# zillow/salve

Hardware: AMD Instinct MI355X
Metric: alignment hypotheses/sec (render+verify) (higher is better)
Workload: dtype fp16

## Files before the change

### include/salve_hip.h

```cpp
#ifndef SALVE_HIP_H
#define SALVE_HIP_H

#include <stddef.h>
#include <stdint.h>

#ifdef __cplusplus
extern "C" {
#endif

typedef enum {
    SALVE_OK = 0,
    SALVE_ERR_BAD_ARG = -1,
    SALVE_ERR_UNSUPPORTED = -2,
    SALVE_ERR_HIP = -3,
    SALVE_ERR_WORKSPACE = -4
} salve_status_t;

#define SALVE_HIP_ABI_VERSION 7

#define SALVE_STATUS_WALK_FAILED 1
#define SALVE_STATUS_FP16_RANGE 2
#define SALVE_STATUS_BAD_HYPOTHESIS 4

#define SALVE_STATUS_LAYOUT_THICKNESS 8
// ... 134 lines not shown

typedef struct {
    int32_t op;
    int32_t in_buf, out_buf, res_buf;
    int32_t Hi, Wi, Cin;
    int32_t Ho, Wo, Cout;
    int32_t KH, KW, stride, pad;
    int32_t relu, reserved;
    int64_t w_off;
    int64_t b_off;
    int64_t ktab_off;
    int32_t in2_buf, Cin2, stride2, Hi2, Wi2, reserved2;
} salve_resnet_op_t;

#define SALVE_RESNET_CONV_IGEMM_ONLY 1
#define SALVE_RESNET_CONV8_WHEREVER 2
#define SALVE_RESNET_ROUND_ROBIN_TILES 4
#define SALVE_RESNET_NO_STEM_FUSE 8
#define SALVE_RESNET_NO_BLOCK_FUSE 16
#define SALVE_RESNET_NO_PROJ_FUSE 32
#define SALVE_RESNET_NO_CHAIN 64
#define SALVE_RESNET_CHAIN_EXPAND_ONLY 128
#define SALVE_RESNET_CHAIN_16_WAVES 256
#define SALVE_RESNET_CHAIN_NO_SPLIT 512
#define SALVE_RESNET_CHAIN_STORE_ALL 1024
#define SALVE_RESNET_NO_TRANSPOSED_TILES 2048
#define SALVE_RESNET_NO_NEXT_FUSE 4096
#define SALVE_RESNET_ALL_FLAGS 8191

void* salve_resnet_create(int32_t num_layers, int32_t in_channels, const salve_resnet_op_t* ops, int32_t n_ops,
                          const void* weights_f16, size_t weights_bytes, const float* params_f32, size_t params_bytes,
                          const int32_t* ktab, size_t ktab_entries, int32_t flags);
void salve_resnet_destroy(void* handle);
int salve_resnet_num_layers(void* handle);
size_t salve_resnet_workspace_bytes(void* handle, int32_t batch);
int salve_resnet_forward(void* handle, const void* input, int32_t batch, float* logits, void* workspace,
                         size_t workspace_bytes, int32_t* status, void* stream);

void* salve_resnet_f32_create(int32_t num_layers, int32_t in_channels, const salve_resnet_op_t* ops, int32_t n_ops,
                              const float* weights_f32, size_t weights_bytes, const float* params_f32, size_t params_bytes,
                              const int32_t* ktab, size_t ktab_entries, int32_t flags);
void salve_resnet_f32_destroy(void* handle);
size_t salve_resnet_f32_workspace_bytes(void* handle, int32_t batch);
int salve_resnet_f32_forward(void* handle, const float* input, int32_t batch, float* logits, void* workspace,
                             size_t workspace_bytes, int32_t* status, void* stream);

typedef struct {
    int32_t batch, Hi, Wi, Cin, Ho, Wo, Cout, KH, KW, stride, pad;
} salve_conv_desc_t;
#define SALVE_CONV_FWD 0
#define SALVE_CONV_DGRAD 1
#define SALVE_CONV_WGRAD 2
size_t salve_conv_f32_workspace_bytes(const salve_conv_desc_t* d, int32_t pass);
int salve_conv_f32_forward(const salve_conv_desc_t* d, const float* x, const float* w, float* y, void* ws, size_t ws_bytes, void* stream);
int salve_conv_f32_backward_data(const salve_conv_desc_t* d, const float* dy, const float* w, float* dx, void* ws, size_t ws_bytes,
                                 void* stream);
int salve_conv_f32_backward_weight(const salve_conv_desc_t* d, const float* x, const float* dy, float* dw, void* ws, size_t ws_bytes,
                                   void* stream);

size_t salve_conv_bf16_workspace_bytes(const salve_conv_desc_t* d, int32_t pass);
int salve_conv_bf16_forward(const salve_conv_desc_t* d, const uint16_t* x, const uint16_t* w, uint16_t* y, void* ws, size_t ws_bytes,
                            void* stream);
int salve_conv_bf16_backward_data(const salve_conv_desc_t* d, const uint16_t* dy, const uint16_t* w, uint16_t* dx, void* ws, size_t ws_bytes,
                                  void* stream);
int salve_conv_bf16_backward_weight(const salve_conv_desc_t* d, const uint16_t* x, const uint16_t* dy, float* dw, void* ws, size_t ws_bytes,
                                    void* stream);
// ... 94 lines not shown
```

### salve_amd/_lib.py

```python

from __future__ import annotations

import ctypes
from pathlib import Path

import numpy as np

import os

LIB_PATH = Path(os.environ.get("SALVE_HIP_LIB") or (Path(__file__).resolve().parent / "libsalve_hip.so"))

SALVE_OK = 0
EXPECTED_ABI = 7
TILE_F32_NCHW = 0
TILE_F16_NHWC = 1
TILE_U8X4 = 2
TILE_F32_NHWC = 3
TILE_BF16_NHWC = 4

EXPORTED_SYMBOLS = (
    "salve_hip_version",
    "salve_last_error",
    "salve_bev_workspace_bytes",
    "salve_bev_pano_index_bytes",
    "salve_bev_pano_index_build",
    "salve_bev_render_batch",
    "salve_bev_scatter",
    "salve_bev_densify",
    "salve_bev_scatter_points",
    "salve_zorder_winners",
    "salve_remove_hallucinated",
    "salve_bev_keys_from_pixels",
    "salve_bev_export_u8",
    "salve_layout_rasterise",
    "salve_bev_tiles",
    "salve_bev_tile_pairs",
    "salve_bev_densify_tiles",
    "salve_resize_rgb_u8",
    "salve_resnet_create",
    "salve_resnet_destroy",
    "salve_resnet_workspace_bytes",
    "salve_resnet_forward",
    "salve_resnet_num_layers",
    "salve_resnet_f32_create",
    "salve_resnet_f32_destroy",
    "salve_resnet_f32_workspace_bytes",
    "salve_resnet_f32_forward",
    "salve_bev_tiles_aug",
    "salve_conv_f32_workspace_bytes",
    "salve_conv_f32_forward",
    "salve_conv_f32_backward_data",
    "salve_conv_f32_backward_weight",
    "salve_conv_bf16_workspace_bytes",
    "salve_conv_bf16_forward",
    "salve_conv_bf16_backward_data",
    "salve_conv_bf16_backward_weight",
    "salve_bn_workspace_bytes",
    "salve_bn_f32_forward",
    "salve_bn_f32_backward",
    "salve_bn_bf16_forward",
    "salve_bn_bf16_backward",
    "salve_bev_train_tiles",
    "salve_bev_pano_index_update",
    "salve_layout_pose",
    "salve_adam_step",
    "salve_head_workspace_bytes",
    "salve_head_f32_forward",
    "salve_head_f32_backward",
    "salve_head_bf16_forward",
    "salve_head_bf16_backward",
    "salve_bev_jpeg_roundtrip_workspace_bytes",
    "salve_bev_jpeg_roundtrip",
    "salve_bev_jpeg_encode_workspace_bytes",
    "salve_bev_jpeg_encode_max_bytes",
    "salve_bev_jpeg_encode",
    "salve_bev_jpeg_decode_workspace_bytes",
# ... 113 lines not shown
    lib.salve_bev_densify.argtypes = [ctypes.POINTER(BevConfig), i32, vp, vp, vp, vp, vp, sz, vp]
    lib.salve_bev_densify.restype = ctypes.c_int
    lib.salve_bev_scatter_points.argtypes = [ctypes.POINTER(BevConfig), vp, vp, i32, vp, vp, vp, sz, vp]
    lib.salve_bev_scatter_points.restype = ctypes.c_int
    lib.salve_zorder_winners.argtypes = [vp, vp, vp, i32, vp, i32, i32, i32, vp, vp, vp]
    lib.salve_zorder_winners.restype = ctypes.c_int
    lib.salve_remove_hallucinated.argtypes = [vp, vp, i32, i32, i32, vp, vp, vp]
    lib.salve_remove_hallucinated.restype = ctypes.c_int
    lib.salve_bev_keys_from_pixels.argtypes = [ctypes.POINTER(BevConfig), vp, vp, i32, vp, vp, sz, vp]
    lib.salve_bev_keys_from_pixels.restype = ctypes.c_int
    lib.salve_layout_rasterise.argtypes = [vp, i32, vp, vp, i32, i32, vp, vp, vp]
    lib.salve_layout_rasterise.restype = ctypes.c_int
    f64, i64 = ctypes.c_double, ctypes.c_int64
    lib.salve_layout_pose.argtypes = [vp, vp, i64, vp, vp, vp, i64, i32, vp, i32, f64, f64, f64, i32, vp, vp, i32, vp, i32, vp, vp]
    lib.salve_layout_pose.restype = ctypes.c_int
    lib.salve_bev_export_u8.argtypes = [vp, i32, i32, i32, vp, vp]
    lib.salve_bev_export_u8.restype = ctypes.c_int
    lib.salve_bev_tiles.argtypes = [vp, i32, i32, vp, i32, vp, vp, i32, i32, vp, vp, i32, i32, vp]
    lib.salve_bev_tiles.restype = ctypes.c_int
    lib.salve_bev_tile_pairs.argtypes = [vp, vp, i32, i32, vp, vp, i32, vp, vp, i32, i32, vp, vp, i32, i32, vp]
    lib.salve_bev_tile_pairs.restype = ctypes.c_int
    lib.salve_bev_densify_tiles.argtypes = [ctypes.POINTER(BevConfig), i32, vp, vp, vp, vp, vp, vp, i32, i32, vp, vp, i32, vp, vp, sz, vp]
    lib.salve_bev_densify_tiles.restype = ctypes.c_int
    lib.salve_resize_rgb_u8.argtypes = [vp, i32, i32, i32, vp, i32, i32, vp, vp, vp]
    lib.salve_resize_rgb_u8.restype = ctypes.c_int
    lib.salve_resnet_create.argtypes = [i32, i32, vp, i32, vp, sz, vp, sz, vp, sz, i32]
    lib.salve_resnet_create.restype = vp
    lib.salve_resnet_destroy.argtypes = [vp]
    lib.salve_resnet_destroy.restype = None
    lib.salve_resnet_workspace_bytes.argtypes = [vp, i32]
    lib.salve_resnet_workspace_bytes.restype = sz
    lib.salve_resnet_forward.argtypes = [vp, vp, i32, vp, vp, sz, vp, vp]
    lib.salve_resnet_forward.restype = ctypes.c_int
    lib.salve_resnet_num_layers.argtypes = [vp]
    lib.salve_resnet_num_layers.restype = ctypes.c_int
    lib.salve_resnet_f32_create.argtypes = [i32, i32, vp, i32, vp, sz, vp, sz, vp, sz, i32]
    lib.salve_resnet_f32_create.restype = vp
    lib.salve_resnet_f32_destroy.argtypes = [vp]
    lib.salve_resnet_f32_destroy.restype = None
    lib.salve_resnet_f32_workspace_bytes.argtypes = [vp, i32]
    lib.salve_resnet_f32_workspace_bytes.restype = sz
    lib.salve_resnet_f32_forward.argtypes = [vp, vp, i32, vp, vp, sz, vp, vp]
    lib.salve_resnet_f32_forward.restype = ctypes.c_int
    lib.salve_bev_tiles_aug.argtypes = [vp, i32, i32, vp, vp, i32, vp, vp, i32, i32, vp, vp, i32, vp]
    lib.salve_bev_tiles_aug.restype = ctypes.c_int
    lib.salve_bev_train_tiles.argtypes = [vp, i32, vp, i32, i32, i32, vp, vp, i32, vp, i32, vp, vp, i32, i32, vp, vp, i32, i32, vp, vp]
    lib.salve_bev_train_tiles.restype = ctypes.c_int
    lib.salve_conv_f32_workspace_bytes.argtypes = [ctypes.POINTER(ConvDesc), i32]
    lib.salve_conv_f32_workspace_bytes.restype = sz
    lib.salve_conv_bf16_workspace_bytes.argtypes = [ctypes.POINTER(ConvDesc), i32]
    lib.salve_conv_bf16_workspace_bytes.restype = sz
    for name in ("salve_conv_f32_forward", "salve_conv_f32_backward_data", "salve_conv_f32_backward_weight", "salve_conv_bf16_forward",
                 "salve_conv_bf16_backward_data", "salve_conv_bf16_backward_weight"):
        getattr(lib, name).argtypes = [ctypes.POINTER(ConvDesc), vp, vp, vp, vp, sz, vp]
        getattr(lib, name).restype = ctypes.c_int
    lib.salve_bn_workspace_bytes.argtypes = [ctypes.POINTER(BnDesc), i32]
    lib.salve_bn_workspace_bytes.restype = sz
    for name in ("salve_bn_f32_forward", "salve_bn_bf16_forward"):
        getattr(lib, name).argtypes = [ctypes.POINTER(BnDesc)] + [vp] * 9 + [vp, sz, vp]
        getattr(lib, name).restype = ctypes.c_int
    for name in ("salve_bn_f32_backward", "salve_bn_bf16_backward"):
        getattr(lib, name).argtypes = [ctypes.POINTER(BnDesc)] + [vp] * 10 + [vp, sz, vp]
        getattr(lib, name).restype = ctypes.c_int
    lib.salve_adam_step.argtypes = [vp, i32, vp, i32, vp, vp, vp]
    lib.salve_adam_step.restype = ctypes.c_int
    lib.salve_head_workspace_bytes.argtypes = [ctypes.POINTER(HeadDesc), i32]
# ... 56 lines not shown
```

### salve_amd/csrc/resnet.hip

```cpp
#include <hip/hip_runtime.h>
#include <stdint.h>
#include <stdlib.h>
#include <string.h>
#include <type_traits>
#include <vector>

#include "../../include/salve_hip.h"
#include "salve_common.h"

namespace {

typedef __attribute__((__ext_vector_type__(8))) _Float16 act8;
typedef __attribute__((__ext_vector_type__(4))) float f32x4;

constexpr int BM = 128;
constexpr int BK = 64;
constexpr int CONV_THREADS = 256;

struct ConvArgs {
    const uint16_t* in;
    const uint16_t* w;
    const float* bias;
    const uint16_t* res;
    uint16_t* out;
// ... 227 lines not shown
    float amin = 0.f;
    const float lo = p.relu ? 0.f : -65504.f;
    float4 bias_j[NT];
#pragma unroll
    for (int j = 0; j < NT; j++) bias_j[j] = *reinterpret_cast<const float4*>(p.bias + n0 + wc * WN + j * 16 + 4 * (lane >> 4));
#pragma unroll
    for (int j = 0; j < NT; j++) {
        const int ncol = wc * WN + j * 16 + 4 * (lane >> 4);
        const float4 bias = bias_j[j];
#pragma unroll
        for (int i = 0; i < 4; i++) {
            const int mrow = wr * 64 + i * 16 + (lane & 15);
            uint2* cell = reinterpret_cast<uint2*>(Cs + mrow * LDC + ncol);
            f32x4 v = acc[i][j] + vec4(bias);
            if (p.res) v += vec4(*cell);
            *cell = pack4_lo(amax, amin, v, lo);
        }
    }

    if (!p.relu) amax = fmaxf(amax, -amin);
    report_range(p.status, amax);
    __syncthreads();
#pragma unroll
    for (int it = 0; it < C_ITERS; it++) {
        if (m0 + crow + it * ROW_STEP < p.M)
            *reinterpret_cast<uint4*>(p.out + coff + it * cstep) = *reinterpret_cast<const uint4*>(Cs + (crow + it * ROW_STEP) * LDC + cch * 8);
    }
}

#ifdef SALVE_BUILD_ABLATIONS
#include "../../tools/probe/ablations/conv_wide.h"
#endif
#include "conv8.h"
#include "stem_pool.h"
#include "expand_chain.h"

__global__ __launch_bounds__(256) void maxpool_kernel(const uint16_t* __restrict__ in, uint16_t* __restrict__ out, int B,
                                                      int Hi, int Wi, int C, int Ho, int Wo) {
    const long long idx = (long long)blockIdx.x * 256 + threadIdx.x;
    const int c8 = C / 8;
    const long long total = (long long)B * Ho * Wo * c8;
    if (idx >= total) return;
    const int ch = (int)(idx % c8);
    long long t = idx / c8;
    const int ox = (int)(t % Wo);
    t /= Wo;
    const int oy = (int)(t % Ho);
    const int b = (int)(t / Ho);
    float best[8];
#pragma unroll
    for (int k = 0; k < 8; k++) best[k] = -3.0e38f;
    for (int dy = 0; dy < 3; dy++) {
        const int iy = oy * 2 - 1 + dy;
        if (iy < 0 || iy >= Hi) continue;
        for (int dx = 0; dx < 3; dx++) {
            const int ix = ox * 2 - 1 + dx;
            if (ix < 0 || ix >= Wi) continue;
            const uint4 v = *reinterpret_cast<const uint4*>(in + (((long long)b * Hi + iy) * Wi + ix) * C + ch * 8);
            const uint32_t w[4] = {v.x, v.y, v.z, v.w};
#pragma unroll
            for (int k = 0; k < 4; k++) {
                best[2 * k] = fmaxf(best[2 * k], act_to_f32((uint16_t)(w[k] & 0xFFFFu)));
                best[2 * k + 1] = fmaxf(best[2 * k + 1], act_to_f32((uint16_t)(w[k] >> 16)));
            }
        }
    }
// ... 498 lines not shown
                const int id = tl + it * BN_THREADS;
                const int m = id / CPR, ch = id % CPR;
                const int oy = img_y(m >> 4, m & 15), ox = img_x(m >> 4, m & 15);
                if (ox < p.W && oy < p.H)
                    store16_stream(timg + ((long long)oy * p.W + ox) * MIDN + ch * 8, *reinterpret_cast<const uint4*>(Cs + m * LDC + ch * 8));
            }
        }
#undef ISSUE_WD
#undef GEMM4_KTILE
    }
    report_range(p.status, amax);
}

struct ResnetHandle {
    std::vector<salve_resnet_op_t> ops;
    uint16_t* d_weights = nullptr;
    float* d_params = nullptr;
    int32_t* d_ktab = nullptr;
    uint16_t* d_zeros = nullptr;
    size_t max_act_elems = 0;
    int n_bufs = 0;
    int num_layers = 0, in_channels = 0, ncls = 0;
    std::vector<int> fused;
    std::vector<int> wide;
    bool wide_auto = false;
    std::vector<int> stem;
    int xcd_contig = 1;
    std::vector<int> chain;
    int n_cus = 256;
    int chain_split = 1;
    int chain_dbg = 0, chain_waves = 8;
    std::vector<int> y_even;
    std::vector<int> next;
    int no_transposed_tiles = 0;
};

static bool chain_shape(int mid, int midn) { return (mid == 128 && (midn == 128 || midn == 256)) || (mid == 256 && midn == 256); }
static bool expand_shape(int mid) { return mid == 128 || mid == 256; }

enum { WIDE_OFF = 0, WIDE_256_K64_S2 = 4, WIDE_128_K64_S1 = 5, WIDE_PC_128 = 6, WIDE_8PHASE = 7, WIDE_AUTO = 8 };

static bool is_pow2(int v) { return v > 0 && (v & (v - 1)) == 0; }

static int choose_wide(const salve_resnet_op_t& o, int force) {
    if (o.op != SALVE_OP_CONV || force == WIDE_OFF) return WIDE_OFF;
    const bool pointwise = o.KH == 1 && o.KW == 1 && o.stride == 1 && o.pad == 0;
    const int K = o.KH * o.KW * o.Cin + (o.in2_buf != SALVE_NO_BUF ? o.Cin2 : 0);
    if (!pointwise && (!is_pow2(o.Cin) || o.Cin < 64)) return WIDE_OFF;
    if (K < 128 || K % 64 != 0) return WIDE_OFF;
    if (force == WIDE_8PHASE || force == WIDE_AUTO) {
        const bool fits = o.Cout % 256 == 0 && is_pow2(o.Cin) && o.Cin >= 64 && (o.in2_buf == SALVE_NO_BUF || o.Cin2 % 64 == 0);
        return (fits && (force == WIDE_8PHASE || K >= 512)) ? WIDE_8PHASE : WIDE_OFF;
    }
    if (force == WIDE_256_K64_S2) return o.Cout % 256 == 0 ? force : WIDE_OFF;
    return o.Cout % 128 == 0 ? force : WIDE_OFF;
}

bool check_op(const salve_resnet_op_t& o) {
    if (o.op == SALVE_OP_CONV) {
        if (o.Cout % 64 != 0) return salve_fail("conv: Cout must be a multiple of 64");
        if (o.Cin % 8 != 0) return salve_fail("conv: Cin must be a multiple of 8");
        if ((o.KH * o.KW * o.Cin) % BK != 0) return salve_fail("conv: KH*KW*Cin must be a multiple of 64");
        if (o.in2_buf != SALVE_NO_BUF) {
            if (o.KH != 1 || o.KW != 1 || o.stride != 1 || o.pad != 0 || o.res_buf != SALVE_NO_BUF)
                return salve_fail("conv: a second source needs a 1x1 / stride 1 / pad 0 convolution without residual");
            if (o.Cin2 <= 0 || o.Cin2 % BK != 0 || o.stride2 < 1 || (o.Hi2 - 1) / o.stride2 + 1 != o.Ho || (o.Wi2 - 1) / o.stride2 + 1 != o.Wo)
// ... 171 lines not shown
        h->chain_split = (flags & SALVE_RESNET_CHAIN_NO_SPLIT) ? 0 : 1;
#ifdef SALVE_BUILD_ABLATIONS
        if (const char* d = getenv("SALVE_CHAIN_DBG")) h->chain_dbg = atoi(d);
#endif
        int dev = 0, cus = 0;
        if (hipGetDevice(&dev) == hipSuccess && hipDeviceGetAttribute(&cus, hipDeviceAttributeMultiprocessorCount, dev) == hipSuccess && cus > 0)
            h->n_cus = cus;
    }
    if (hipMalloc(&h->d_weights, weights_bytes) != hipSuccess || hipMalloc(&h->d_params, params_bytes) != hipSuccess ||
        hipMalloc(&h->d_ktab, ktab_entries * sizeof(int32_t)) != hipSuccess || hipMalloc(&h->d_zeros, 256) != hipSuccess) {
        salve_fail("salve_resnet_create: hipMalloc failed");
        salve_resnet_destroy(h);
        return nullptr;
    }
    if (hipMemcpy(h->d_weights, weights_f16, weights_bytes, hipMemcpyHostToDevice) != hipSuccess ||
        hipMemcpy(h->d_params, params_f32, params_bytes, hipMemcpyHostToDevice) != hipSuccess ||
        hipMemcpy(h->d_ktab, ktab, ktab_entries * sizeof(int32_t), hipMemcpyHostToDevice) != hipSuccess ||
        hipMemset(h->d_zeros, 0, 256) != hipSuccess) {
        salve_fail("salve_resnet_create: hipMemcpy failed");
        salve_resnet_destroy(h);
        return nullptr;
    }
    return h;
}

void salve_resnet_destroy(void* handle) {
    ResnetHandle* h = reinterpret_cast<ResnetHandle*>(handle);
    if (!h) return;
    if (h->d_weights) (void)hipFree(h->d_weights);
    if (h->d_params) (void)hipFree(h->d_params);
    if (h->d_ktab) (void)hipFree(h->d_ktab);
    if (h->d_zeros) (void)hipFree(h->d_zeros);
    delete h;
}

int salve_resnet_num_layers(void* handle) { return handle ? reinterpret_cast<ResnetHandle*>(handle)->num_layers : 0; }

size_t salve_resnet_workspace_bytes(void* handle, int32_t batch) {
    ResnetHandle* h = reinterpret_cast<ResnetHandle*>(handle);
    if (!h || batch <= 0) return 0;
    return (size_t)h->n_bufs * (size_t)batch * h->max_act_elems * sizeof(uint16_t) + 256;
}

int salve_resnet_forward(void* handle, const void* input, int32_t batch, float* logits, void* workspace,
                         size_t workspace_bytes, int32_t* status, void* stream) {
    ResnetHandle* h = reinterpret_cast<ResnetHandle*>(handle);
    if (!h || !input || !logits || !workspace || batch <= 0) {
        salve_fail("salve_resnet_forward: null argument or bad batch");
        return SALVE_ERR_BAD_ARG;
    }
    if (workspace_bytes < salve_resnet_workspace_bytes(handle, batch)) {
        salve_fail("salve_resnet_forward: workspace too small");
        return SALVE_ERR_WORKSPACE;
    }
    hipStream_t s = (hipStream_t)stream;
    uint16_t* base = reinterpret_cast<uint16_t*>(((uintptr_t)workspace + 255) & ~(uintptr_t)255);
    const size_t buf_elems = (size_t)batch * h->max_act_elems;
    auto buf = [&](int i) -> uint16_t* { return i < 0 ? const_cast<uint16_t*>(reinterpret_cast<const uint16_t*>(input)) : base + (size_t)i * buf_elems; };
    for (size_t oi = 0; oi < h->ops.size(); oi++) {
        const salve_resnet_op_t& o = h->ops[oi];
        if (o.op == SALVE_OP_CONV && h->stem[oi]) {
            const salve_resnet_op_t& pool = h->ops[oi + 1];
            StemArgs a;
            a.x = buf(o.in_buf);
            a.w = h->d_weights + o.w_off;
            a.bias = h->d_params + o.b_off;
// ... 88 lines not shown
            a.ktab = h->d_ktab + o.ktab_off;
            a.zeros = h->d_zeros;
            a.status = status;
            a.xcd_contig = h->xcd_contig;
            a.B = batch; a.Hi = o.Hi; a.Wi = o.Wi; a.Cin = o.Cin; a.Ho = o.Ho; a.Wo = o.Wo; a.Cout = o.Cout;
            a.stride = o.stride; a.pad = o.pad; a.K = o.KH * o.KW * o.Cin; a.relu = o.relu;
            const bool src2 = o.in2_buf != SALVE_NO_BUF;
            a.in2 = src2 ? buf(o.in2_buf) : nullptr;
            a.Hi2 = o.Hi2; a.Wi2 = o.Wi2; a.Cin2 = o.Cin2; a.stride2 = o.stride2;
            a.nkt1 = a.K / BK;
            if (src2) a.K += o.Cin2;
            const long long M = (long long)batch * o.Ho * o.Wo;
            if (M > 0x7FFFFFFFll) { salve_fail("batch too large"); return SALVE_ERR_BAD_ARG; }
            a.M = (int)M;
            a.KW = o.KW;
            a.cin_log2 = 0;
            while ((1 << a.cin_log2) < o.Cin) a.cin_log2++;
            const bool few_tiles = h->wide[oi] == WIDE_8PHASE && h->wide_auto && ((M + 255) / 256) * (long long)(o.Cout / 256) < 1536;
            if (h->wide[oi] != WIDE_OFF && !few_tiles) {
                const int cfg = h->wide[oi];
                const int bn = (cfg == WIDE_256_K64_S2 || cfg == WIDE_8PHASE) ? 256 : 128;
                a.m_tiles = (int)((M + C8_BM - 1) / C8_BM);
                a.n_tiles = o.Cout / bn;
                const unsigned grid = (unsigned)(((a.m_tiles + 7) / 8) * 8 * a.n_tiles);
                const bool pw = o.KH == 1 && o.KW == 1 && o.stride == 1 && o.pad == 0;
#ifdef SALVE_BUILD_ABLATIONS
#define WIDE_LAUNCH(BN_, KS_, NS_)                                                                                                  \
    {                                                                                                                               \
        if (src2) hipLaunchKernelGGL((conv_wide_kernel<BN_, KS_, NS_, true, true>), dim3(grid), dim3(WIDE_THREADS), 0, s, a);       \
        else if (pw) hipLaunchKernelGGL((conv_wide_kernel<BN_, KS_, NS_, true, false>), dim3(grid), dim3(WIDE_THREADS), 0, s, a);   \
        else hipLaunchKernelGGL((conv_wide_kernel<BN_, KS_, NS_, false, false>), dim3(grid), dim3(WIDE_THREADS), 0, s, a);          \
    }
#endif
                if (cfg == WIDE_8PHASE) {
                    if (src2) hipLaunchKernelGGL((conv8_kernel<true, true>), dim3(grid), dim3(C8_THREADS), 0, s, a);
                    else if (pw) hipLaunchKernelGGL((conv8_kernel<true, false>), dim3(grid), dim3(C8_THREADS), 0, s, a);
                    else hipLaunchKernelGGL((conv8_kernel<false, false>), dim3(grid), dim3(C8_THREADS), 0, s, a);
                }
#ifdef SALVE_BUILD_ABLATIONS
                else if (cfg == WIDE_PC_128) {
                    if (src2) hipLaunchKernelGGL((conv_pc_kernel<true, true>), dim3(grid), dim3(PC_THREADS), 0, s, a);
                    else if (pw) hipLaunchKernelGGL((conv_pc_kernel<true, false>), dim3(grid), dim3(PC_THREADS), 0, s, a);
                    else hipLaunchKernelGGL((conv_pc_kernel<false, false>), dim3(grid), dim3(PC_THREADS), 0, s, a);
                } else if (cfg == WIDE_256_K64_S2) WIDE_LAUNCH(256, 64, 2)
                else WIDE_LAUNCH(128, 64, 1)
#undef WIDE_LAUNCH
#endif
                SALVE_HIP_CHECK(hipGetLastError());
                continue;
            }
            a.m_tiles = (int)((M + BM - 1) / BM);
            const int bn = (o.Cout % 128 == 0) ? 128 : 64;
            a.n_tiles = o.Cout / bn;
            const unsigned grid = (unsigned)(((a.m_tiles + 7) / 8) * 8 * a.n_tiles);
            const bool pointwise = o.KH == 1 && o.KW == 1 && o.stride == 1 && o.pad == 0;
            if (src2 && bn == 128) {
                hipLaunchKernelGGL((conv_igemm_kernel<128, true, true>), dim3(grid), dim3(CONV_THREADS), 0, s, a);
            } else if (src2) {
                hipLaunchKernelGGL((conv_igemm_kernel<64, true, true>), dim3(grid), dim3(CONV_THREADS), 0, s, a);
            } else if (bn == 128 && pointwise) {
                hipLaunchKernelGGL((conv_igemm_kernel<128, true>), dim3(grid), dim3(CONV_THREADS), 0, s, a);
            } else if (bn == 128) {
                hipLaunchKernelGGL((conv_igemm_kernel<128, false>), dim3(grid), dim3(CONV_THREADS), 0, s, a);
            } else if (pointwise) {
                hipLaunchKernelGGL((conv_igemm_kernel<64, true>), dim3(grid), dim3(CONV_THREADS), 0, s, a);
            } else {
                hipLaunchKernelGGL((conv_igemm_kernel<64, false>), dim3(grid), dim3(CONV_THREADS), 0, s, a);
// ... 16 lines not shown
```

### salve_amd/models/hip_resnet.py

```python

from __future__ import annotations

import ctypes
from typing import Dict, List, Tuple

import numpy as np
import torch

from salve_amd import _lib, status
from salve_amd.models.resnet_factory import RESNET_SPECS

OP_CONV, OP_MAXPOOL, OP_AVGPOOL_FC = 0, 1, 2
NET_INPUT, NO_BUF = -1, -2
BN_EPS = 1e-5

OP_DTYPE = np.dtype(
    [("op", "<i4"), ("in_buf", "<i4"), ("out_buf", "<i4"), ("res_buf", "<i4"), ("Hi", "<i4"), ("Wi", "<i4"),
     ("Cin", "<i4"), ("Ho", "<i4"), ("Wo", "<i4"), ("Cout", "<i4"), ("KH", "<i4"), ("KW", "<i4"), ("stride", "<i4"),
     ("pad", "<i4"), ("relu", "<i4"), ("reserved", "<i4"), ("w_off", "<i8"), ("b_off", "<i8"), ("ktab_off", "<i8"),
     ("in2_buf", "<i4"), ("Cin2", "<i4"), ("stride2", "<i4"), ("Hi2", "<i4"), ("Wi2", "<i4"), ("reserved2", "<i4")]
)
assert OP_DTYPE.itemsize == 112


# ... 130 lines not shown
                    b.conv1x1_with_shortcut(wc, bc, t2, outb, Ho, Wo, wd, bd, x, H, W, stride)
                else:
                    b.conv(wc, bc, t2, outb, x, Ho, Wo, 1, 0, True)
            else:
                wa, ba = fold_bn(sd[f"{p}.conv1.weight"], _bn(sd, f"{p}.bn1"))
                wb, bb = fold_bn(sd[f"{p}.conv2.weight"], _bn(sd, f"{p}.bn2"))
                Ho, Wo = b.conv(wa, ba, x, t1, NO_BUF, H, W, stride, 1, True)
                idn = x
                if f"{p}.downsample.0.weight" in sd:
                    wd, bd = fold_bn(sd[f"{p}.downsample.0.weight"], _bn(sd, f"{p}.downsample.1"))
                    b.conv(wd, bd, x, dsb, NO_BUF, H, W, stride, 0, False)
                    idn = dsb
                b.conv(wb, bb, t1, outb, idn, Ho, Wo, 1, 1, True)
            x, H, W = outb, Ho, Wo
    feat = sd["fc.weight"].shape[1]
    b.fc(sd["fc.weight"], sd["fc.bias"], x, H, W, feat)
    ops = np.array(b.ops, dtype=OP_DTYPE)
    if precision == "fp32":
        weights = np.concatenate(b.weights).astype(np.float32)
        for arr, what in ((weights, "convolution weights (after folding BatchNorm)"), (np.concatenate(b.params), "biases / fc parameters")):
            if not np.isfinite(arr).all():
                raise ValueError(f"checkpoint has non-finite {what}")
        return ops, weights, np.concatenate(b.params).astype(np.float32), np.concatenate(b.ktab).astype(np.int32), cin_p
    for arr, what in ((np.concatenate(b.weights).astype(np.int16).view(np.float16), "convolution weights (after folding BatchNorm)"),
                      (np.concatenate(b.params), "biases / fc parameters")):
        if not np.isfinite(arr.astype(np.float32)).all():
            raise ValueError(f"checkpoint has non-finite {what}, or values beyond the fp16 range")
    return ops, np.concatenate(b.weights).astype(np.int16), np.concatenate(b.params).astype(np.float32), \
        np.concatenate(b.ktab).astype(np.int32), cin_p


class HipResNet:

    def __init__(self, state_dict: Dict[str, torch.Tensor], num_layers: int, device: torch.device, flags: int = 0) -> None:
        self.lib = _lib.load()
        self.device = torch.device(device)
        if self.device.type != "cuda":
            raise _lib.SalveHipError("HipResNet needs a HIP device ('cuda:N'); there is no CPU path")
        ops, wbits, params, ktab, cin_p = build_program(state_dict, num_layers)
        self.in_channels = cin_p
        self.num_classes = int(ops[-1]["Cout"])
        self.n_ops = len(ops)
        with torch.cuda.device(self.device):
            h = self.lib.salve_resnet_create(
                num_layers, cin_p, ops.ctypes.data_as(ctypes.c_void_p), len(ops),
                wbits.ctypes.data_as(ctypes.c_void_p), wbits.nbytes, params.ctypes.data_as(ctypes.c_void_p), params.nbytes,
                ktab.ctypes.data_as(ctypes.c_void_p), ktab.size, int(flags),
            )
        if not h:
            _lib.check(-1, "salve_resnet_create")
        self.handle = ctypes.c_void_p(h)
        self._ws = None

    def __del__(self) -> None:
        try:
            if getattr(self, "handle", None):
                self.lib.salve_resnet_destroy(self.handle)
                self.handle = None
        except Exception:
            pass

    def forward_nhwc(self, x: torch.Tensor, out: torch.Tensor = None) -> torch.Tensor:
        assert x.dtype == torch.float16 and x.is_contiguous() and x.shape[-1] == self.in_channels, (x.dtype, x.shape)
        B = int(x.shape[0])
        need = self.lib.salve_resnet_workspace_bytes(self.handle, B)
        if self._ws is None or self._ws.numel() < need:
            self._ws = torch.empty(need, dtype=torch.uint8, device=self.device)
        if out is None:
            out = torch.empty((B, self.num_classes), dtype=torch.float32, device=self.device)
        with torch.cuda.device(self.device):
            st = self.lib.salve_resnet_forward(
                self.handle, ctypes.c_void_p(x.data_ptr()), B, ctypes.c_void_p(out.data_ptr()),
                ctypes.c_void_p(self._ws.data_ptr()), self._ws.numel(), status.ptr(self.device),
                ctypes.c_void_p(torch.cuda.current_stream(self.device).cuda_stream),
            )
        _lib.check(st, "salve_resnet_forward")
        return out


class HipResNetF32:

    def __init__(self, state_dict: Dict[str, torch.Tensor], num_layers: int, device: torch.device, flags: int = 0) -> None:
        self.lib = _lib.load()
        self.device = torch.device(device)
        if self.device.type != "cuda":
# ... 60 lines not shown
```

Before: 60780.

## Add four-wave conv8 variant with 8x8 MFMA tiles per wave for spatial convs

Adds a 256-thread (4-wave) version of the 8-phase fp16 conv kernel in which each wave owns a 128x128 slice and holds an 8x8 grid of 16x16 MFMA accumulators. It keeps the swizzled LDS ring and direct global-to-LDS loads and pins one wave per EU. By default it is used for non-pointwise convs, selectable per handle through a new setter. The aim is more reuse of fragments per LDS read and fewer waves to synchronise, at the cost of very high register pressure and lower occupancy.

After: 61160, median of 6. Within noise of the previous version (+0.6%).

```diff
diff --git a/include/salve_hip.h b/include/salve_hip.h
--- a/include/salve_hip.h
+++ b/include/salve_hip.h
@@ -190,6 +190,7 @@
                           const void* weights_f16, size_t weights_bytes, const float* params_f32, size_t params_bytes,
                           const int32_t* ktab, size_t ktab_entries, int32_t flags);
 void salve_resnet_destroy(void* handle);
+int salve_resnet_set_conv8_waves(void* handle, int32_t waves);
 int salve_resnet_num_layers(void* handle);
 size_t salve_resnet_workspace_bytes(void* handle, int32_t batch);
 int salve_resnet_forward(void* handle, const void* input, int32_t batch, float* logits, void* workspace,
diff --git a/salve_amd/_lib.py b/salve_amd/_lib.py
--- a/salve_amd/_lib.py
+++ b/salve_amd/_lib.py
@@ -42,6 +42,7 @@
     "salve_resnet_workspace_bytes",
     "salve_resnet_forward",
     "salve_resnet_num_layers",
+    "salve_resnet_set_conv8_waves",
     "salve_resnet_f32_create",
     "salve_resnet_f32_destroy",
     "salve_resnet_f32_workspace_bytes",
@@ -221,6 +222,8 @@
     lib.salve_resnet_workspace_bytes.restype = sz
     lib.salve_resnet_forward.argtypes = [vp, vp, i32, vp, vp, sz, vp, vp]
     lib.salve_resnet_forward.restype = ctypes.c_int
+    lib.salve_resnet_set_conv8_waves.argtypes = [vp, i32]
+    lib.salve_resnet_set_conv8_waves.restype = ctypes.c_int
     lib.salve_resnet_num_layers.argtypes = [vp]
     lib.salve_resnet_num_layers.restype = ctypes.c_int
     lib.salve_resnet_f32_create.argtypes = [i32, i32, vp, i32, vp, sz, vp, sz, vp, sz, i32]
diff --git a/salve_amd/csrc/conv8w.h b/salve_amd/csrc/conv8w.h
--- /dev/null
+++ b/salve_amd/csrc/conv8w.h
@@ -0,0 +1,227 @@
+
+constexpr int C8W_THREADS = 256;
+
+template <bool POINTWISE, bool SRC2>
+__global__ __launch_bounds__(C8W_THREADS) __attribute__((amdgpu_waves_per_eu(1, 1))) void conv8w_kernel(ConvArgs p) {
+    constexpr int BM = C8_BM, BN = C8_BN, KS = C8_KS;
+    constexpr int LDC = BN + 8;
+    constexpr int RING_E = 8 * C8_HALF_E, C_E = BM * LDC;
+    __shared__ __attribute__((aligned(1024))) uint16_t smem[RING_E > C_E ? RING_E : C_E];
+
+    int m_tile, n_tile;
+    if (!xcd_tile(blockIdx.x, p.m_tiles, p.n_tiles, p.xcd_contig, m_tile, n_tile)) return;
+    const int tid = threadIdx.x, lane = tid & 63, wave = __builtin_amdgcn_readfirstlane(tid >> 6);
+    const int wr = wave >> 1, wc = wave & 1;
+    const int m0 = m_tile * BM, n0 = n_tile * BN;
+    const int r8 = tid >> 3;
+    const int chunk = (tid & 7) ^ ((r8 >> 1) & 7);
+
+#define C8W_ROW(S, I) (((I) >> 1) * 128 + (S) * 64 + ((I) & 1) * 32)
+    int iyx0[2][4];
+    const uint16_t* rowp[2][4];
+    const uint16_t* rowp2[2][4];
+#pragma unroll
+    for (int s = 0; s < 2; s++)
+#pragma unroll
+        for (int i = 0; i < 4; i++) {
+            const int m = m0 + C8W_ROW(s, i) + r8;
+            const bool valid = m < p.M;
+            rowp[s][i] = nullptr;
+            rowp2[s][i] = nullptr;
+            iyx0[s][i] = 0;
+            if (SRC2 && valid) {
+                const int ox = m % p.Wo, t = m / p.Wo, oy = t % p.Ho, b = t / p.Ho;
+                rowp2[s][i] = p.in2 + (((long long)b * p.Hi2 + (long long)oy * p.stride2) * p.Wi2 + (long long)ox * p.stride2) * p.Cin2 + chunk * 8;
+            }
+            if (POINTWISE) {
+                rowp[s][i] = valid ? p.in + (long long)m * p.Cin + chunk * 8 : nullptr;
+            } else {
+                const int mm = valid ? m : 0;
+                const int ox = mm % p.Wo, t = mm / p.Wo, oy = t % p.Ho, b = t / p.Ho;
+                const int iy0 = valid ? oy * p.stride - p.pad : -20000;
+                const int ix0 = ox * p.stride - p.pad;
+                iyx0[s][i] = (int)(((unsigned)iy0 << 16) | ((unsigned)ix0 & 0xFFFFu));
+                rowp[s][i] = p.in + (((long long)b * p.Hi + (valid ? iy0 : 0)) * p.Wi + ix0) * p.Cin + chunk * 8;
+            }
+        }
+    const uint16_t* wbase = p.w + (long long)(n0 + r8) * p.K + chunk * 8;
+
+    const int nkt = p.K / KS;
+
+#define C8W_SLOT(PAR, KIND) (smem + ((((PAR) & 1) << 2) + (KIND)) * C8_HALF_E)
+#define C8W_STAGE_BEGIN(KT, PAR, KIND)                                                                                 \
+    uint16_t* const dst_ = C8W_SLOT(PAR, KIND) + wave * 8 * KS;                                                        \
+    const int kt_ = (KT);                                                                                              \
+    const bool live_ = kt_ < nkt;                                                                                      \
+    int dy_ = 0, dx_ = 0, delta_ = 0;                                                                                  \
+    if (!POINTWISE && ((KIND) == 0 || (KIND) == 3)) {                                                                  \
+        const int k0_ = kt_ * KS;                                                                                      \
+        const int tap_ = k0_ >> p.cin_log2;                                                                            \
+        dy_ = tap_ / p.KW;                                                                                             \
+        dx_ = tap_ - dy_ * p.KW;                                                                                       \
+        delta_ = (dy_ * p.Wi + dx_) * p.Cin + (k0_ & (p.Cin - 1));                                                     \
+    }
+#define C8W_STAGE_ONE(KIND, I)                                                                                         \
+    {                                                                                                                  \
+        constexpr int s_ = ((KIND) == 2 || (KIND) == 3) ? 1 : 0;                                                       \
+        const uint16_t* src = p.zeros;                                                                                 \
+        if ((KIND) == 0 || (KIND) == 3) {                                                                              \
+            if (live_) {                                                                                               \
+                if (SRC2 && kt_ >= p.nkt1) {                                                                           \
+                    if (rowp2[s_][I]) src = rowp2[s_][I] + (kt_ - p.nkt1) * KS;                                        \
+                } else if (POINTWISE) {                                                                                \
+                    if (rowp[s_][I]) src = rowp[s_][I] + kt_ * KS;                                                     \
+                } else if ((unsigned)((iyx0[s_][I] >> 16) + dy_) < (unsigned)p.Hi &&                                   \
+                           (unsigned)((int)(short)iyx0[s_][I] + dx_) < (unsigned)p.Wi) {                               \
+                    src = rowp[s_][I] + delta_;                                                                        \
+                }                                                                                                      \
+            }                                                                                                          \
+        } else if (live_) {                                                                                            \
+            src = wbase + (long long)C8W_ROW(s_, I) * p.K + kt_ * KS;                                                  \
+        }                                                                                                              \
+        __builtin_amdgcn_global_load_lds((global_cptr)src, (lds_ptr)(dst_ + (I) * 32 * KS), 16, 0, 0);                 \
+    }
+#define C8W_STAGE(KT, PAR, KIND)                                                                                       \
+    {                                                                                                                  \
+        C8W_STAGE_BEGIN(KT, PAR, KIND)                                                                                 \
+        _Pragma("unroll") for (int i = 0; i < 4; i++) C8W_STAGE_ONE(KIND, i)                                           \
+    }
+
+    f32x4 acc[8][8];
+#pragma unroll
+    for (int i = 0; i < 8; i++)
+#pragma unroll
+        for (int j = 0; j < 8; j++) acc[i][j] = f32x4{0.f, 0.f, 0.f, 0.f};
+
+    const int frag_row = lane & 15, frag_q = lane >> 4;
+    const int frag_sw = (frag_row >> 1) & 7;
+    const int a_off = (wr * 64 + frag_row) * KS, b_off = (wc * 64 + frag_row) * KS;
+    const int pos0 = ((0 * 4 + frag_q) ^ frag_sw) * 8, pos1 = ((1 * 4 + frag_q) ^ frag_sw) * 8;
+
+    act8 fa0[4][2], fa1[4][2], fbp[4][2], fbq[4][2];
+#define C8W_READ(DST, PAR, KIND, OFF)                                                                                  \
+    {                                                                                                                  \
+        const uint16_t* h_ = C8W_SLOT(PAR, KIND) + (OFF);                                                              \
+        _Pragma("unroll") for (int i = 0; i < 4; i++) {                                                                \
+            DST[i][0] = *reinterpret_cast<const act8*>(h_ + i * 16 * KS + pos0);                                       \
+            DST[i][1] = *reinterpret_cast<const act8*>(h_ + i * 16 * KS + pos1);                                       \
+        }                                                                                                              \
+    }
+#define C8W_MFMA(B_, A_, C_) asm volatile("v_mfma_f32_16x16x32_f16 %0, %1, %2, %0" : "+a"(C_) : "v"(B_), "v"(A_) : "memory");
+#define C8W_LANDED(WAIT, DST)                                                                                          \
+    asm volatile(WAIT : "+v"(DST[0][0]), "+v"(DST[0][1]), "+v"(DST[1][0]), "+v"(DST[1][1]), "+v"(DST[2][0]), "+v"(DST[2][1]), \
+                        "+v"(DST[3][0]), "+v"(DST[3][1]) : : "memory");
+#define C8W_READ_ONE(DST, R) DST[(R) & 3][(R) >> 2] = *reinterpret_cast<const act8*>(h_ + ((R) & 3) * 16 * KS + (((R) >> 2) ? pos1 : pos0));
+#define C8W_PHASE(QA, AF, QB, BF, RDST, RPAR, RKIND, ROFF, SKT, SPAR, SKIND)                                           \
+    {                                                                                                                  \
+        C8W_STAGE_BEGIN(SKT, SPAR, SKIND)                                                                              \
+        const uint16_t* h_ = C8W_SLOT(RPAR, RKIND) + (ROFF);                                                           \
+        _Pragma("unroll") for (int ks = 0; ks < 2; ks++)                                                               \
+            _Pragma("unroll") for (int i = 0; i < 4; i++) {                                                            \
+                _Pragma("unroll") for (int j = 0; j < 4; j++) C8W_MFMA(BF[j][ks], AF[i][ks], acc[(QA) * 4 + i][(QB) * 4 + j]) \
+                const int g = ks * 4 + i;                                                                              \
+                if (g < 4) { C8W_READ_ONE(RDST, 2 * g) C8W_READ_ONE(RDST, 2 * g + 1) }                                 \
+                if (g >= 3 && g <= 6) C8W_STAGE_ONE(SKIND, g - 3)                                                      \
+            }                                                                                                          \
+        C8W_LANDED("s_waitcnt vmcnt(16) lgkmcnt(0)", RDST)                                                             \
+        __builtin_amdgcn_s_barrier();                                                                                  \
+        __builtin_amdgcn_sched_barrier(0);                                                                             \
+    }
+#define C8W_KTILE(KT, PAR, BP, BQ)                                                                                     \
+    {                                                                                                                  \
+        C8W_PHASE(0, fa0, 0, BP, BQ, PAR, 2, b_off, (KT) + 1, (PAR) + 1, 3)            \
+        C8W_PHASE(0, fa0, 1, BQ, fa1, PAR, 3, a_off, (KT) + 2, PAR, 0)                 \
+        C8W_PHASE(1, fa1, 1, BQ, fa0, (PAR) + 1, 0, a_off, (KT) + 2, PAR, 1)           \
+        C8W_PHASE(1, fa1, 0, BP, BQ, (PAR) + 1, 1, b_off, (KT) + 2, PAR, 2)            \
+    }
+
+    C8W_STAGE(0, 0, 0);
+    C8W_STAGE(0, 0, 1);
+    C8W_STAGE(0, 0, 2);
+    C8W_STAGE(0, 0, 3);
+    C8W_STAGE(1, 1, 0);
+    C8W_STAGE(1, 1, 1);
+    C8W_STAGE(1, 1, 2);
+    asm volatile("s_waitcnt vmcnt(16)" ::: "memory");
+    __builtin_amdgcn_s_barrier();
+    C8W_READ(fa0, 0, 0, a_off);
+    C8W_READ(fbp, 0, 1, b_off);
+    C8W_LANDED("s_waitcnt lgkmcnt(0)", fa0)
+    C8W_LANDED("s_waitcnt lgkmcnt(0)", fbp)
+    int kt = 0;
+    for (; kt + 1 < nkt; kt += 2) {
+        C8W_KTILE(kt, 0, fbp, fbq);
+        C8W_KTILE(kt + 1, 1, fbq, fbp);
+    }
+    if (kt < nkt) C8W_KTILE(kt, 0, fbp, fbq);
+#undef C8W_STAGE
+#undef C8W_STAGE_BEGIN
+#undef C8W_STAGE_ONE
+#undef C8W_READ
+#undef C8W_MFMA
+#undef C8W_LANDED
+#undef C8W_PHASE
+#undef C8W_READ_ONE
+#undef C8W_KTILE
+#undef C8W_SLOT
+#undef C8W_ROW
+    asm volatile("s_waitcnt vmcnt(0)\n\ts_nop 15" ::: "memory");
+    __builtin_amdgcn_s_barrier();
+    __builtin_amdgcn_sched_barrier(0);
+
+    uint16_t* Cs = smem;
+    constexpr int CH_PER_ROW = BN / 8;
+    constexpr int C_ITERS = (BM * CH_PER_ROW) / C8W_THREADS;
+    constexpr int ROW_STEP = C8W_THREADS / CH_PER_ROW;
+    const int crow = tid / CH_PER_ROW, cch = tid % CH_PER_ROW;
+    const long long coff = (long long)(m0 + crow) * p.Cout + n0 + cch * 8;
+    const int cstep = ROW_STEP * p.Cout;
+    float4 bias_v[8];
+#pragma unroll
+    for (int j = 0; j < 8; j++) bias_v[j] = *reinterpret_cast<const float4*>(p.bias + n0 + wc * 128 + j * 16 + 4 * frag_q);
+    if (p.res) {
+        constexpr int RB = 8;
+#pragma unroll
+        for (int it0 = 0; it0 < C_ITERS; it0 += RB) {
+            uint4 rv[RB];
+#pragma unroll
+            for (int u = 0; u < RB; u++) {
+                const bool in = m0 + crow + (it0 + u) * ROW_STEP < p.M;
+                rv[u] = *reinterpret_cast<const uint4*>(p.res + (in ? coff + (long long)(it0 + u) * cstep : (long long)m0 * p.Cout + n0));
+            }
+#pragma unroll
+            for (int u = 0; u < RB; u++)
+                *reinterpret_cast<uint4*>(Cs + (crow + (it0 + u) * ROW_STEP) * LDC + cch * 8) = rv[u];
+        }
+        __syncthreads();
+    }
+    float amax = 0.f;
+    float amin = 0.f;
+    const float lo = p.relu ? 0.f : -65504.f;
+#define C8W_CELL(I, J) reinterpret_cast<uint2*>(Cs + (wr * 128 + (I) * 16 + frag_row) * LDC + wc * 128 + (J) * 16 + 4 * frag_q)
+#define C8W_PACK(RES)                                                                                                  \
+    {                                                                                                                  \
+        uint2 rr[2][8];                                                                                                \
+        if (RES) { _Pragma("unroll") for (int i = 0; i < 8; i++) rr[0][i] = *C8W_CELL(i, 0); }                         \
+        _Pragma("unroll") for (int j = 0; j < 8; j++) {                                                                \
+            if (RES && j < 7) { _Pragma("unroll") for (int i = 0; i < 8; i++) rr[(j + 1) & 1][i] = *C8W_CELL(i, j + 1); } \
+            _Pragma("unroll") for (int i = 0; i < 8; i++) {                                                            \
+                asm volatile("" : "+a"(acc[i][j]));                                                                    \
+                f32x4 v = acc[i][j] + vec4(bias_v[j]);                                                                 \
+                if (RES) v += vec4(rr[j & 1][i]);                                                                      \
+                *C8W_CELL(i, j) = pack4_lo(amax, amin, v, lo);                                                         \
+            }                                                                                                          \
+        }                                                                                                              \
+    }
+    if (p.res) C8W_PACK(true) else C8W_PACK(false)
+#undef C8W_PACK
+#undef C8W_CELL
+    if (!p.relu) amax = fmaxf(amax, -amin);
+    report_range(p.status, amax);
+    __syncthreads();
+#pragma unroll 4
+    for (int it = 0; it < C_ITERS; it++) {
+        if (m0 + crow + it * ROW_STEP < p.M)
+            *reinterpret_cast<uint4*>(p.out + coff + (long long)it * cstep) = *reinterpret_cast<const uint4*>(Cs + (crow + it * ROW_STEP) * LDC + cch * 8);
+    }
+}
diff --git a/salve_amd/csrc/resnet.hip b/salve_amd/csrc/resnet.hip
--- a/salve_amd/csrc/resnet.hip
+++ b/salve_amd/csrc/resnet.hip
@@ -283,6 +283,7 @@
 #include "../../tools/probe/ablations/conv_wide.h"
 #endif
 #include "conv8.h"
+#include "conv8w.h"
 #include "stem_pool.h"
 #include "expand_chain.h"
 
@@ -847,6 +848,7 @@
     int chain_dbg = 0, chain_waves = 8;
     std::vector<int> y_even;
     std::vector<int> next;
+    int conv8_waves = 0;
     int no_transposed_tiles = 0;
 };
 
@@ -1084,6 +1086,16 @@
     if (h->d_ktab) (void)hipFree(h->d_ktab);
     if (h->d_zeros) (void)hipFree(h->d_zeros);
     delete h;
+}
+
+int salve_resnet_set_conv8_waves(void* handle, int32_t waves) {
+    ResnetHandle* h = reinterpret_cast<ResnetHandle*>(handle);
+    if (!h || (waves != 0 && waves != 4 && waves != 8)) {
+        salve_fail("salve_resnet_set_conv8_waves: a handle and 0 (by shape), 4 or 8 waves");
+        return SALVE_ERR_BAD_ARG;
+    }
+    h->conv8_waves = waves;
+    return SALVE_OK;
 }
 
 int salve_resnet_num_layers(void* handle) { return handle ? reinterpret_cast<ResnetHandle*>(handle)->num_layers : 0; }
@@ -1238,7 +1250,12 @@
         else hipLaunchKernelGGL((conv_wide_kernel<BN_, KS_, NS_, false, false>), dim3(grid), dim3(WIDE_THREADS), 0, s, a);          \
     }
 #endif
-                if (cfg == WIDE_8PHASE) {
+                const bool four_waves = h->conv8_waves == 4 || (h->conv8_waves == 0 && !pw);
+                if (cfg == WIDE_8PHASE && four_waves && o.Hi < 16384 && o.Wi < 16384 && o.pad < 16384) {
+                    if (src2) hipLaunchKernelGGL((conv8w_kernel<true, true>), dim3(grid), dim3(C8W_THREADS), 0, s, a);
+                    else if (pw) hipLaunchKernelGGL((conv8w_kernel<true, false>), dim3(grid), dim3(C8W_THREADS), 0, s, a);
+                    else hipLaunchKernelGGL((conv8w_kernel<false, false>), dim3(grid), dim3(C8W_THREADS), 0, s, a);
+                } else if (cfg == WIDE_8PHASE) {
                     if (src2) hipLaunchKernelGGL((conv8_kernel<true, true>), dim3(grid), dim3(C8_THREADS), 0, s, a);
                     else if (pw) hipLaunchKernelGGL((conv8_kernel<true, false>), dim3(grid), dim3(C8_THREADS), 0, s, a);
                     else hipLaunchKernelGGL((conv8_kernel<false, false>), dim3(grid), dim3(C8_THREADS), 0, s, a);
diff --git a/salve_amd/models/hip_resnet.py b/salve_amd/models/hip_resnet.py
--- a/salve_amd/models/hip_resnet.py
+++ b/salve_amd/models/hip_resnet.py
@@ -186,7 +186,8 @@
 
 class HipResNet:
 
-    def __init__(self, state_dict: Dict[str, torch.Tensor], num_layers: int, device: torch.device, flags: int = 0) -> None:
+    def __init__(self, state_dict: Dict[str, torch.Tensor], num_layers: int, device: torch.device, flags: int = 0,
+                 conv8_waves: int = None) -> None:
         self.lib = _lib.load()
         self.device = torch.device(device)
         if self.device.type != "cuda":
@@ -205,6 +206,8 @@
             _lib.check(-1, "salve_resnet_create")
         self.handle = ctypes.c_void_p(h)
         self._ws = None
+        if conv8_waves is not None:
+            _lib.check(self.lib.salve_resnet_set_conv8_waves(self.handle, int(conv8_waves)), "salve_resnet_set_conv8_waves")
 
     def __del__(self) -> None:
         try:
```
